# sidward14/gan-lab

Measured on AMD Instinct MI355X. Metric: images/sec (G+D step), StyleGAN 1024^2 bs32/GPU, higher is better.
Workload: dtype f32; 1 GPU; StyleGAN res_samples=1024 FFHQ-shaped synthetic, bs=32/GPU fp32, nonsaturating + R1(lambda=10) + drift, stabilised phase, 1 D-iter + 1 G-iter; global_batch=32, per_gpu_batch=32, parallelism=single

## Files before the change

### gan_lab_amd/csrc/common.h

```cpp
#pragma once
#include <hip/hip_runtime.h>
#include <stdint.h>

#include "../../include/ganlab_hip.h"

typedef float f32x4 __attribute__((ext_vector_type(4)));

static thread_local int gl_launch_status = GANLAB_OK;
extern thread_local const void* gl_last_kernel_fn;
extern thread_local unsigned gl_last_grid;
#define GL_LAUNCH_RING 16
extern thread_local const void* gl_ring_fn[GL_LAUNCH_RING];
extern thread_local unsigned gl_ring_grid[GL_LAUNCH_RING];
extern thread_local unsigned long long gl_launch_count;
#define GL_LAUNCH(k, grid, ...)                                                  \
  do {                                                                           \
    (void)hipGetLastError();                                                     \
    const dim3 gl_grid_ = (grid);                                                \
    gl_last_kernel_fn = reinterpret_cast<const void*>(k);                        \
    gl_last_grid = gl_grid_.x * gl_grid_.y * gl_grid_.z;                         \
    gl_ring_fn[gl_launch_count % GL_LAUNCH_RING] = gl_last_kernel_fn;            \
    gl_ring_grid[gl_launch_count % GL_LAUNCH_RING] = gl_last_grid;               \
    ++gl_launch_count;                                                           \
    hipLaunchKernelGGL(k, gl_grid_, __VA_ARGS__);                                \
    if (hipGetLastError() != hipSuccess) gl_launch_status = GANLAB_ELAUNCH;      \
  } while (0)
static inline int gl_take_status() {
  const int s = gl_launch_status;
  gl_launch_status = GANLAB_OK;
  return s;
}
#define GL_CHECK_LAUNCH() gl_take_status()

#include <cstdlib>
#define GL_ENV_ONCE(name) ([]() -> const char* { static const char* const v = getenv(name); return v; }())

static inline hipStream_t gl_stream(void* s) { return reinterpret_cast<hipStream_t>(s); }

__device__ __forceinline__ int gl_xcd_remap(int b, int n) {
  const int q = n >> 3, r = n & 7, xcd = b & 7, i = b >> 3;
  const int base = (xcd < r) ? xcd * (q + 1) : r * (q + 1) + (xcd - r) * q;
  return base + i;
}

__device__ __forceinline__ float gl_wave_sum(float v) {
#pragma unroll
  for (int o = 32; o > 0; o >>= 1) v += __shfl_xor(v, o, 64);
  return v;
}

__device__ __forceinline__ float gl_block_sum_256(float v, float* red) {
  v = gl_wave_sum(v);
  __syncthreads();
  if ((threadIdx.x & 63) == 0) red[threadIdx.x >> 6] = v;
  __syncthreads();
  return red[0] + red[1] + red[2] + red[3];
}

__device__ __forceinline__ double gl_block_sum_256d(double v, double* red) {
#pragma unroll
  for (int o = 32; o > 0; o >>= 1) v += __shfl_xor(v, o, 64);
  __syncthreads();
  if ((threadIdx.x & 63) == 0) red[threadIdx.x >> 6] = v;
  __syncthreads();
  return (red[0] + red[1]) + (red[2] + red[3]);
}

#ifndef GL_ACC_DUMP
#define GL_ACC_DUMP 1
#endif
#ifndef GL_ACC_DUMP_TERMS_V
#define GL_ACC_DUMP_TERMS_V 144
#endif
constexpr int GL_ACC_DUMP_TERMS = GL_ACC_DUMP_TERMS_V;

__device__ __forceinline__ void philox4x32_10(uint32_t c[4], uint32_t k0, uint32_t k1) {
#pragma unroll
  for (int r = 0; r < 10; ++r) {
    const uint64_t p0 = (uint64_t)0xD2511F53u * c[0], p1 = (uint64_t)0xCD9E8D57u * c[2];
    const uint32_t n0 = (uint32_t)(p1 >> 32) ^ c[1] ^ k0, n1 = (uint32_t)p1;
    const uint32_t n2 = (uint32_t)(p0 >> 32) ^ c[3] ^ k1, n3 = (uint32_t)p0;
    c[0] = n0; c[1] = n1; c[2] = n2; c[3] = n3;
    k0 += 0x9E3779B9u;
    k1 += 0xBB67AE85u;
  }
}

__device__ __forceinline__ float gl_lrelu(float v, float slope) { return v > 0.f ? v : v * slope; }

__device__ __forceinline__ float4 gl_few_dot(const float4 (&xv)[4], const float* __restrict__ wp, int Cin, int Cout_p, int co,
                                             float start) {
  float4 a = float4{start, start, start, start};
#pragma unroll
  for (int ci = 0; ci < 4; ++ci) {
    const float w = ci < Cin ? wp[(long long)ci * Cout_p + co] : 0.f;
    a.x += w * xv[ci].x; a.y += w * xv[ci].y; a.z += w * xv[ci].z; a.w += w * xv[ci].w;
  }
  return a;
}

struct gl_bf16x3 { __bf16 h, m, l; };
__device__ __forceinline__ gl_bf16x3 gl_split3(float v) {
  const __bf16 h = (__bf16)v;
  const float r1 = v - (float)h;
  const __bf16 m = (__bf16)r1;
  return gl_bf16x3{h, m, (__bf16)(r1 - (float)m)};
}

__device__ __forceinline__ void gl_x3_pack_position(const float* __restrict__ w9, bool flip, float scale, __bf16* __restrict__ out,
                                                    int CI, int ci, int co) {
  const int steps = CI / 32 * 9;
  const int ct = co >> 6, col = co & 63, c = ci >> 5, half = (ci >> 4) & 1, g = (ci >> 3) & 1, j = ci & 7;
#pragma unroll
  for (int t = 0; t < 9; ++t) {
    const int s = t < 8 ? (half ? 5 : 0) + (t >> 1) : 4;
    const int hi = t < 8 ? (t & 1) : half;
    const int kg = hi * 2 + g;
    float v = w9[flip ? 8 - t : t] * scale;
    asm volatile("" : "+v"(v));
    const gl_bf16x3 p = gl_split3(v);
    __bf16* base = out + (((long long)ct * steps + c * 9 + s) * (3 * 4 * 64)) * 8;
    base[((0 * 4 + kg) * 64 + col) * 8 + j] = p.h;
    base[((1 * 4 + kg) * 64 + col) * 8 + j] = p.m;
    base[((2 * 4 + kg) * 64 + col) * 8 + j] = p.l;
  }
}

__device__ __forceinline__ void gl_x3_up_pack_position(const float* __restrict__ w9, int up, float scale, __bf16* __restrict__ out,
                                                       int CI, int CO, int ci, int co) {
  const int nsteps = CI / 8;
  const bool c32 = (CO & 63) != 0;
  const int ct = c32 ? co >> 5 : co >> 6, j = ci & 7;
#pragma unroll
  for (int py = 0; py < 2; ++py)
#pragma unroll
    for (int px = 0; px < 2; ++px)
#pragma unroll
      for (int ty = 0; ty < 2; ++ty)
#pragma unroll
        for (int tx = 0; tx < 2; ++tx) {
          float v = 0.f;
#pragma unroll
          for (int ky = 0; ky < 3; ++ky)
#pragma unroll
            for (int kx = 0; kx < 3; ++kx) {
              const int ry = up ? ky : 2 - ky, rx = up ? kx : 2 - kx;
              const bool iny = py == 0 ? (ty == 0 ? ry == 0 : ry >= 1) : (ty == 0 ? ry <= 1 : ry == 2);
              const bool inx = px == 0 ? (tx == 0 ? rx == 0 : rx >= 1) : (tx == 0 ? rx <= 1 : rx == 2);
              if (iny && inx) v += w9[ky * 3 + kx];
            }
          v = v * (up ? scale : 0.25f * scale);
          asm volatile("" : "+v"(v));
          const gl_bf16x3 p = gl_split3(v);
          __bf16* base = out + (((c32 ? (long long)ct : (long long)ct * 2 + py) * nsteps + (ci >> 3)) * (3 * 4 * 128)) * 8;
          const int col = c32 ? py * 32 + (co & 31) : co & 63;
          const int kgq = ty * 2 + tx;
          base[((0 * 4 + kgq) * 128 + px * 64 + col) * 8 + j] = p.h;
          base[((1 * 4 + kgq) * 128 + px * 64 + col) * 8 + j] = p.m;
          base[((2 * 4 + kgq) * 128 + px * 64 + col) * 8 + j] = p.l;
        }
}

__device__ __forceinline__ float gl_comb_s2(int up, int a, int k) {
  if (up) {
    const int lo = (a == 0) ? 2 : (a == 1 ? 1 : 0), hi = (a == 0) ? 2 : (a == 1 ? 2 : (a == 2 ? 1 : 0));
    return (k >= lo && k <= hi) ? 1.f : 0.f;
  }
  const int lo = (a <= 1) ? 0 : (a == 2 ? 1 : 2), hi = (a == 0) ? 0 : (a == 1 ? 1 : 2);
  return (k >= lo && k <= hi) ? 0.5f : 0.f;
}
__device__ __forceinline__ void gl_x3_down_pack_position(const float* __restrict__ w9, int up, float scale, __bf16* __restrict__ out,
                                                         int CI, int ci, int co) {
  const int nsteps = CI / 8 * 4;
  const int ct = co >> 7, col = co & 127, q = ci >> 3, j = ci & 7;
  float k9[9];
#pragma unroll
  for (int t = 0; t < 9; ++t) k9[t] = w9[t];
#pragma unroll
  for (int a = 0; a < 4; ++a)
#pragma unroll
    for (int b = 0; b < 4; ++b) {
      float v = 0.f;
#pragma unroll
      for (int ky = 0; ky < 3; ++ky)
#pragma unroll
        for (int kx = 0; kx < 3; ++kx) v += gl_comb_s2(up, a, ky) * gl_comb_s2(up, b, kx) * k9[ky * 3 + kx];
      v = v * scale;
      asm volatile("" : "+v"(v));
      const gl_bf16x3 p = gl_split3(v);
      __bf16* base = out + (((long long)ct * nsteps + q * 4 + a) * (3 * 4 * 128)) * 8;
      base[((0 * 4 + b) * 128 + col) * 8 + j] = p.h;
      base[((1 * 4 + b) * 128 + col) * 8 + j] = p.m;
      base[((2 * 4 + b) * 128 + col) * 8 + j] = p.l;
    }
}

extern "C" int gl_tail_stats_finish(const double* spart, float* mean, float* rstd, long long planes, int chunks, double inv_hw, float eps,
                         hipStream_t st);

bool gl_wgrad_roll_supported(int N, int Cin, int Cout, int H, int W, int ks, int pad, int up, const void* x,
                             const void* gy);
int gl_wgrad_roll_slots(int N, int Cin, int Cout, int H, int W);
int gl_wgrad_roll_launch(const float* x, const float* gy, float* part, int N, int Cin, int Cout, int H, int W,
                         hipStream_t st, const float* aff_s = nullptr, const float* aff_t = nullptr);
bool gl_wgrad_s2_roll_supported(int N, int Cl, int Ch, int Hl, int Wl, const void* low, const void* high);
int gl_wgrad_s2_roll_slots(int N, int Cl, int Ch, int Hl, int Wl);
int gl_wgrad_s2_roll_launch(const float* low, const float* high, float* part, int N, int Cl, int Ch, int Hl, int Wl,
                            hipStream_t st, const float* aff_s = nullptr, const float* aff_t = nullptr);

bool gl_s2_roll_supported(int is_T, int N, int Cin, int Cout, int Hl, int Wl, const void* x, const void* y);
int gl_s2_roll_launch(int is_T, const float* x, const float* wp, const float* bias, float* y, int N, int Cin, int Cout,
                      int Hl, int Wl, int Cin_p, int Cout_p, float bias_scale, int act, float slope, hipStream_t st,
                      const float* aff_s = nullptr, const float* aff_t = nullptr);

bool gl_roll_blur_supported(int N, int Cin, int Cout, int H, int W, const void* x, const void* y);
int gl_roll_blur_launch(const float* x, const float* wp, const float* bias, float* y, void* bits, int N, int Cin, int Cout,
                        int H, int W, int Cin_p, int Cout_p, float bias_scale, float slope, hipStream_t st, int blur, int act);
```

### gan_lab_amd/csrc/conv_x3_down.hip

```cpp
#include "x3_common.h"

#include <type_traits>

namespace {

constexpr int XD_NT = 128;
constexpr int XD_PP = 160;
constexpr int XD_PL = 4 * XD_PP;
constexpr int XD_Q = 3 * XD_PL;
constexpr int XD_WSTEP = 3 * 4 * XD_NT;
constexpr int XD_WOFF = 3 * XD_Q;
constexpr int XD_LDS = 3 * XD_Q + 2 * XD_WSTEP;

#define XD_ACC8(a) "+v"(a[0][0]), "+v"(a[0][1]), "+v"(a[0][2]), "+v"(a[0][3]), "+v"(a[1][0]), "+v"(a[1][1]), "+v"(a[1][2]), "+v"(a[1][3])

struct XDArgs {
  const float* x;
  const u32x4* wp;
  const float* bias;
  float* y;
  int N, CI, CO, Hl, Wl;
  int tiles_x, tiles_y, tiles_co, ntiles;
  float bias_scale, slope;
  int act;
};
struct XDTile { int n, oy0, ox0, co_t; };

__global__ __launch_bounds__(512) void conv_x3_down_kernel(XDArgs p) {
  __shared__ __attribute__((aligned(16))) u32x4 lds[XD_LDS];
  const int tid = threadIdx.x, lane = tid & 63;
  const int wv = __builtin_amdgcn_readfirstlane(tid >> 6);
  const int wm = wv >> 1, wn = wv & 1;
  const int l16 = lane & 15, kg = lane >> 4, lane16 = lane * 16;
  const int Hi = 2 * p.Hl, Wi = 2 * p.Wl;
  const int plane = Hi * Wi;
  const int oplane = p.Hl * p.Wl;
  const int nq = p.CI / 8;
  const int G = gridDim.x;

  auto decode = [&](int t) {
    XDTile c;
    c.co_t = t % p.tiles_co; t /= p.tiles_co;
    c.ox0 = (t % p.tiles_x) * 16; t /= p.tiles_x;
    c.oy0 = (t % p.tiles_y) * 8;
    c.n = t / p.tiles_y;
    return c;
  };

  const bool a_item = tid < 360;
  int a_r, a_cg, a_cq;
  {
    const int e = a_item ? tid : 0;
    a_cq = e & 1;
    const int t = e >> 1;
    a_cg = t % 10;
    a_r = t / 10;
  }
  const int cstride = plane * 4;
  f32x4 arA[4], arB[4];
  auto a_load_to = [&](f32x4 (&ar)[4], const XDTile& c, int q) {
    const u32x4 rs = x3_rsrc(p.x + (long long)c.n * p.CI * plane, (unsigned)((long long)p.CI * plane * 4));
    int r = a_r;
    asm volatile("" : "+v"(r));
    const int iy = 2 * c.oy0 - 1 + r, ix = 2 * c.ox0 - 4 + 4 * a_cg;
    const bool ok = a_item && (unsigned)iy < (unsigned)Hi && (unsigned)ix < (unsigned)Wi;
    const int off = ok ? ((a_cq * 4) * plane + iy * Wi + ix) * 4 : (int)0x80000000;
    const int soff = q * 8 * plane * 4;
#pragma unroll
    for (int j = 0; j < 4; ++j) x3_ld(ar[j], rs, off + j * cstride, soff);
  };
  auto a_store_from = [&](const f32x4 (&ar)[4], int slot, int i) {
    if (!a_item) return;
    int r = a_r;
    asm volatile("" : "+v"(r));
    const int c = 4 * a_cg - 3 + i;
    if (c < 0 || c > 33) return;
    bf16x4 h, m, l;
#pragma unroll
    for (int j = 0; j < 4; ++j) x3_split_lane(ar[j][i], j, h, m, l);
    const int unit = slot * XD_Q + ((r & 1) * 2 + (c & 1)) * XD_PP + (r >> 1) * 17 + (c >> 1);
    unsigned char* dst = reinterpret_cast<unsigned char*>(lds + unit) + a_cq * 8;
    *reinterpret_cast<u32x2*>(dst) = __builtin_bit_cast(u32x2, h);
    *reinterpret_cast<u32x2*>(dst + XD_PL * 16) = __builtin_bit_cast(u32x2, m);
    *reinterpret_cast<u32x2*>(dst + 2 * XD_PL * 16) = __builtin_bit_cast(u32x2, l);
  };
  auto a_load = [&](int set, const XDTile& c, int q) { if (set == 0) a_load_to(arA, c, q); else a_load_to(arB, c, q); };
  auto a_store_px = [&](int set, int slot, int i) { if (set == 0) a_store_from(arA, slot, i); else a_store_from(arB, slot, i); };
  auto a_wait = [&](int set, auto younger) {
    constexpr int Y = decltype(younger)::value;
    if (set == 0) x3_ld_wait<Y>(arA); else x3_ld_wait<Y>(arB);
  };

  const int nsteps = nq * 4;
  const __amdgpu_buffer_rsrc_t rs_w = __builtin_amdgcn_make_buffer_rsrc(
      const_cast<u32x4*>(p.wp), 0, (unsigned)((long long)p.tiles_co * nsteps * XD_WSTEP * 16), 0x00020000);
  auto w_dma = [&](const XDTile& c, int step, int buf) {
    const int soff = (c.co_t * nsteps + step) * (XD_WSTEP * 16) + wv * 3072;
#pragma unroll
    for (int i = 0; i < 3; ++i)
      __builtin_amdgcn_raw_ptr_buffer_load_lds(rs_w, (__attribute__((address_space(3))) void*)(lds + XD_WOFF + buf * XD_WSTEP + wv * 192 + i * 64),
                                               16, lane16, soff + i * 1024, 0, 0);
  };

  f32x4 accS[2][4], accH[2][4], accT[2][4];
#pragma unroll
  for (int m = 0; m < 2; ++m)
#pragma unroll
    for (int nn = 0; nn < 4; ++nn) {
      accS[m][nn] = f32x4{0.f, 0.f, 0.f, 0.f}; accH[m][nn] = f32x4{0.f, 0.f, 0.f, 0.f}; accT[m][nn] = f32x4{0.f, 0.f, 0.f, 0.f};
    }
  X3_SETTLE(XD_ACC8(accS));
  X3_SETTLE(XD_ACC8(accH));

  const int laneA = (kg & 1) * XD_PP + (2 * wm) * 17 + l16 + (kg >> 1);
  const int laneB = XD_WOFF + kg * XD_NT + wn * 64 + l16;

  bf16x8 aF[2][2][3];
  bf16x8 bF[2][3];
  auto a_frags = [&](int off, int set) {
#pragma unroll
    for (int m = 0; m < 2; ++m)
#pragma unroll
      for (int pl = 0; pl < 3; ++pl) aF[set][m][pl] = __builtin_bit_cast(bf16x8, lds[laneA + off + pl * XD_PL + m * 17]);
  };
  auto b_frags = [&](int buf, int nn, int set) {
#pragma unroll
    for (int pl = 0; pl < 3; ++pl) bF[set][pl] = __builtin_bit_cast(bf16x8, lds[laneB + buf * XD_WSTEP + pl * 4 * XD_NT + nn * 16]);
  };

  int tile = gl_xcd_remap(blockIdx.x, G);
  if (tile >= p.ntiles) return;
  XDTile cur = decode(tile);
  int sa = 0, sb = 1, sc = 2;

  w_dma(cur, 0, 0);
  a_load(0, cur, 0);
  a_wait(0, std::integral_constant<int, 0>{});
#pragma unroll
  for (int i = 0; i < 4; ++i) { a_store_px(0, sa, i); __builtin_amdgcn_sched_barrier(0); }
  x3_barrier<0>();
  w_dma(cur, 1, 1);
  __builtin_amdgcn_sched_barrier(0);
  a_load(1, cur, 1);
  a_wait(1, std::integral_constant<int, 0>{});
  a_frags(sa * XD_Q, 0);
  b_frags(0, 0, 0);

  int q = 0, gs = 0;
  for (;;) {
    const int ntile = tile + G;
    const bool nvalid = ntile < p.ntiles;
    const XDTile nxt = decode(nvalid ? ntile : tile);
    for (; q < nq; q += 2) {
#pragma unroll
      for (int s8 = 0; s8 < 8; ++s8) {
        const int qq = q + (s8 >> 2), a = s8 & 3;
        const int buf = (gs + s8) & 1, cs = s8 & 1;
        const int setn = (s8 >> 2) ^ 1;
        const bool has_next = a < 3 || qq + 1 < nq || nvalid;
        const bool next_q = qq + 1 < nq || nvalid;
        const int offN = a < 3 ? sa * XD_Q + ((a + 1) & 1) * 2 * XD_PP + ((a + 1) >> 1) * 17 : sb * XD_Q;
#pragma unroll
        for (int nn = 0; nn < 4; ++nn) {
          if (nn < 3) b_frags(buf, nn + 1, (nn + 1) & 1);
          if (nn == 3) {
            if (a == 1 && (qq + 2 < nq || nvalid)) x3_barrier<4>(); else x3_barrier<0>();
            {
              const int st2 = qq * 4 + a + 2;
              if (st2 < nsteps) w_dma(cur, st2, buf);
              else if (nvalid) w_dma(nxt, st2 - nsteps, buf);
            }
            __builtin_amdgcn_sched_barrier(0);
            if (a == 0) {
              if (qq + 2 < nq) a_load(setn ^ 1, cur, qq + 2);
              else if (nvalid) a_load(setn ^ 1, nxt, qq + 2 - nq);
            }
            if (has_next) { a_frags(offN, cs ^ 1); b_frags(buf ^ 1, 0, 0); }
          }
          __builtin_amdgcn_sched_barrier(0);
#pragma unroll
          for (int m = 0; m < 2; ++m) {
            X3_MFMA(accS[m][nn], aF[cs][m][2], bF[nn & 1][0]);
            X3_MFMA(accS[m][nn], aF[cs][m][0], bF[nn & 1][2]);
            X3_MFMA(accS[m][nn], aF[cs][m][1], bF[nn & 1][1]);
            X3_MFMA(accS[m][nn], aF[cs][m][1], bF[nn & 1][0]);
            X3_MFMA(accS[m][nn], aF[cs][m][0], bF[nn & 1][1]);
            X3_MFMA(accH[m][nn], aF[cs][m][0], bF[nn & 1][0]);
          }
          __builtin_amdgcn_sched_barrier(0);
          if (nn == 1 && next_q) {
            if (a == 0) a_wait(setn, std::integral_constant<int, 9>{});
            a_store_px(setn, sb, a);
            __builtin_amdgcn_sched_barrier(0);
          }
        }
        if (a == 3) { const int t_ = sa; sa = sb; sb = sc; sc = t_; }
      }
      gs += 8;
      X3_DRAIN(XD_ACC8(accH));
#pragma unroll
      for (int m = 0; m < 2; ++m)
#pragma unroll
        for (int nn = 0; nn < 4; ++nn) { accT[m][nn] += accH[m][nn]; accH[m][nn] = f32x4{0.f, 0.f, 0.f, 0.f}; }
      X3_SETTLE(XD_ACC8(accH));
      __builtin_amdgcn_sched_barrier(0);
    }

    {
      X3_DRAIN(XD_ACC8(accS));
      typedef const __attribute__((address_space(4))) XDArgs* XDArgsK;
      unsigned long long kpi = (unsigned long long)__builtin_amdgcn_kernarg_segment_ptr();
      asm volatile("" : "+s"(kpi));
      const XDArgsK kp = (XDArgsK)kpi;
      float* const y = kp->y;
      const float* const bias = kp->bias;
      const float bias_scale = kp->bias_scale, slope = kp->slope;
      const int act = kp->act;
      const long long ib = (long long)cur.n * p.CO * oplane;
#pragma unroll
      for (int nn = 0; nn < 4; ++nn) {
        const int co = cur.co_t * XD_NT + wn * 64 + nn * 16 + l16;
        const float bv = bias != nullptr ? bias[co] * bias_scale : 0.f;
#pragma unroll
        for (int m = 0; m < 2; ++m) {
          f32x4 v = accT[m][nn] + accS[m][nn];
#pragma unroll
          for (int r = 0; r < 4; ++r) {
            float f = v[r] + bv;
            if (act == GANLAB_ACT_LRELU) f = gl_lrelu(f, slope);
            v[r] = f;
          }
          *reinterpret_cast<f32x4*>(y + ib + (long long)co * oplane + (cur.oy0 + 2 * wm + m) * p.Wl + cur.ox0 + 4 * kg) = v;
          accT[m][nn] = f32x4{0.f, 0.f, 0.f, 0.f};
          accS[m][nn] = f32x4{0.f, 0.f, 0.f, 0.f};
        }
      }
      X3_SETTLE(XD_ACC8(accS));
    }
    if (!nvalid) break;
    tile = ntile;
    cur = nxt;
    q = 0;
  }
}

__global__ void x3_down_pack_kernel(const float* __restrict__ w, __bf16* __restrict__ out, int Cout, int Cin, int up, float scale) {
  const int CO = up ? Cin : Cout, CI = up ? Cout : Cin;
  const long long e = blockIdx.x * (long long)blockDim.x + threadIdx.x;
  if (e >= (long long)CO * CI) return;
  const int col = (int)(e & 127);
  const long long t = e >> 7;
  const int ci = (int)(t % CI), ct = (int)(t / CI);
  const int co = ct * 128 + col;
  const float* w9 = up ? w + ((long long)ci * Cin + co) * 9 : w + ((long long)co * Cin + ci) * 9;
  gl_x3_down_pack_position(w9, up, scale, out, CI, ci, co);
}

long long xd_tiles(int N, int CI, int CO, int Hl, int Wl) {
  const long long ntiles = (long long)N * (Wl / 16) * (Hl / 8) * (CO / XD_NT);
  const bool fits = ntiles > 0 && ntiles <= 0x7fffffffLL && (long long)(CO / XD_NT) * (CI / 8 * 4) * XD_WSTEP * 16 <= 0xffffffffLL &&
                    (long long)CI * Hl * Wl * 16 <= 0x7fffffffLL;
  return fits ? ntiles : 0;
}

bool xd_ok(const ganlab_conv_geom* g, int dgrad) {
  if (g == nullptr || g->ks != 3 || g->pad != 1 || g->N <= 0) return false;
  if (dgrad ? !(g->up == 1 && g->pool == 0) : !(g->pool == 1 && g->up == 0)) return false;
  const int CI = dgrad ? g->Cout : g->Cin, CO = dgrad ? g->Cin : g->Cout;
  if (!dgrad && ((g->Hin | g->Win) & 1)) return false;
  const int Hl = dgrad ? g->Hin : g->Hin / 2, Wl = dgrad ? g->Win : g->Win / 2;
  if (!(CI % 16 == 0 && CO % XD_NT == 0 && Hl % 8 == 0 && Wl % 16 == 0)) return false;
  return xd_tiles(g->N, CI, CO, Hl, Wl) > 0;
}

int xd_launch(const float* x, const void* wp, const float* bias, float* y, int N, int CI, int CO, int Hl, int Wl, float bias_scale,
              int act, float slope, hipStream_t st) {
  XDArgs a{};
  a.x = x; a.wp = reinterpret_cast<const u32x4*>(wp); a.bias = bias; a.y = y;
  a.N = N; a.CI = CI; a.CO = CO; a.Hl = Hl; a.Wl = Wl;
  a.tiles_x = Wl / 16; a.tiles_y = Hl / 8; a.tiles_co = CO / XD_NT;
  a.bias_scale = bias_scale; a.slope = slope; a.act = act;
  const long long ntiles = xd_tiles(N, CI, CO, Hl, Wl);
  if (ntiles <= 0) return GANLAB_EINVAL;
  a.ntiles = (int)ntiles;
  const unsigned grid = (unsigned)(ntiles < 256 ? ntiles : 256);
  GL_LAUNCH(conv_x3_down_kernel, dim3(grid), dim3(512), 0, st, a);
  return GL_CHECK_LAUNCH();
}

}

extern "C" {

int ganlab_conv_s2_down_x3_supported(const ganlab_conv_geom* g, int dgrad) { return xd_ok(g, dgrad) ? 1 : 0; }

long long ganlab_conv_s2_down_x3_pack(const float* w, void* out, int Cout, int Cin, int up, float scale, void* stream) {
  if (Cout <= 0 || Cin <= 0 || (up != 0 && up != 1)) return GANLAB_EINVAL;
  const int CO = up ? Cin : Cout, CI = up ? Cout : Cin;
  if (CO % XD_NT != 0 || CI % 16 != 0) return GANLAB_EINVAL;
  const long long n = 48LL * Cout * Cin;
  if (out == nullptr) return n;
  if (w == nullptr) return GANLAB_EINVAL;
  const long long positions = (long long)Cout * Cin;
  GL_LAUNCH(x3_down_pack_kernel, dim3((unsigned)((positions + 255) / 256)), dim3(256), 0, gl_stream(stream), w,
            reinterpret_cast<__bf16*>(out), Cout, Cin, up, scale);
  const int st = GL_CHECK_LAUNCH();
  return st != GANLAB_OK ? st : n;
}

int ganlab_conv_s2_down_fwd_x3(const float* x, const void* wp, const float* bias, float* y, const ganlab_conv_geom* g,
                               float bias_scale, int act, float slope, void* stream) {
  if (!xd_ok(g, 0) || x == nullptr || wp == nullptr || y == nullptr) return GANLAB_EINVAL;
  return xd_launch(x, wp, bias, y, g->N, g->Cin, g->Cout, g->Hin / 2, g->Win / 2, bias_scale, act, slope, gl_stream(stream));
}

int ganlab_conv_s2_down_dgrad_x3(const float* gy, const void* wp, float* gx, const ganlab_conv_geom* g, void* stream) {
  if (!xd_ok(g, 1) || gy == nullptr || wp == nullptr || gx == nullptr) return GANLAB_EINVAL;
  return xd_launch(gy, wp, nullptr, gx, g->N, g->Cout, g->Cin, g->Hin, g->Win, 1.f, GANLAB_ACT_NONE, 0.f, gl_stream(stream));
}

}
```

### gan_lab_amd/csrc/pack.hip

```cpp
#include "common.h"

namespace {

constexpr int round_up_c(int v, int m) { return (v + m - 1) / m * m; }

__global__ __launch_bounds__(256) void pack_many_kernel(const ganlab_pack_desc* __restrict__ descs, int n_desc) {
  int lo = 0, hi = n_desc - 1;
  const long long b = blockIdx.x;
  while (lo < hi) {
    const int mid = (lo + hi + 1) >> 1;
    if (descs[mid].block0 <= b) lo = mid; else hi = mid - 1;
  }
  const ganlab_pack_desc d = descs[lo];
  const long long e = (b - d.block0) * 256 + threadIdx.x;
  const float* w = d.src;
  if (d.kind == GANLAB_PACKKIND_PLAIN) {
    const int KK = d.ks * d.ks, dgrad = d.mode == GANLAB_PACK_DGRAD;
    const int rows = dgrad ? d.Cout : d.Cin, cols = dgrad ? d.Cin : d.Cout;
    const int rows_p = round_up_c(rows, d.ks == 1 ? 32 : 16), cols_p = round_up_c(cols, 64);
    const long long plane = (long long)rows_p * cols_p;
    if (e >= plane) return;
    const int col = (int)(e % cols_p), row = (int)(e / cols_p);
    const bool in = row < rows && col < cols;
    const int co = dgrad ? row : col, ci = dgrad ? col : row;
    const float* ws = w + ((long long)co * d.Cin + ci) * KK;
    float* out = reinterpret_cast<float*>(d.dst) + e;
    for (int tap = 0; tap < KK; ++tap)
      out[tap * plane] = in ? d.scale * ws[dgrad ? (KK - 1 - tap) : tap] : 0.f;
  } else if (d.kind == GANLAB_PACKKIND_S2) {
    const int transpose = d.mode;
    const int rows = transpose ? d.Cout : d.Cin, cols = transpose ? d.Cin : d.Cout;
    const int rows_p = round_up_c(rows, 16), cols_p = round_up_c(cols, 64);
    const long long plane = (long long)rows_p * cols_p;
    if (e >= plane) return;
    const int col = (int)(e % cols_p), row = (int)(e / cols_p);
    const bool in = row < rows && col < cols;
    const int co = transpose ? row : col, ci = transpose ? col : row;
    float k9[9];
    const float* ws = w + ((long long)co * d.Cin + ci) * 9;
#pragma unroll
    for (int t = 0; t < 9; ++t) k9[t] = in ? ws[t] : 0.f;
    float* out = reinterpret_cast<float*>(d.dst) + e;
#pragma unroll
    for (int tap = 0; tap < 16; ++tap) {
      const int a = tap >> 2, bb = tap & 3;
      float v = 0.f;
#pragma unroll
      for (int ky = 0; ky < 3; ++ky)
#pragma unroll
        for (int kx = 0; kx < 3; ++kx) v += gl_comb_s2(d.up, a, ky) * gl_comb_s2(d.up, bb, kx) * k9[ky * 3 + kx];
      out[tap * plane] = v * d.scale;
    }
  } else if (d.kind == GANLAB_PACKKIND_X3 && d.ks == 4) {
    const int up = d.up;
    const int CO = up ? d.Cout : d.Cin, CI = up ? d.Cin : d.Cout;
    if (e >= (long long)CO * CI) return;
    int ci, co;
    if ((CO & 63) == 0) {
      const int col = (int)(e & 63);
      const long long t = e >> 6;
      ci = (int)(t % CI);
      co = (int)(t / CI) * 64 + col;
    } else {
      co = (int)(e % CO);
      ci = (int)(e / CO);
    }
    const float* w9 = up ? w + ((long long)co * d.Cin + ci) * 9 : w + ((long long)ci * d.Cin + co) * 9;
    gl_x3_up_pack_position(w9, up, d.scale, reinterpret_cast<__bf16*>(d.dst), CI, CO, ci, co);
  } else if (d.kind == GANLAB_PACKKIND_X3 && d.ks == 5) {
    const int up = d.up;
    const int CO = up ? d.Cin : d.Cout, CI = up ? d.Cout : d.Cin;
    if (e >= (long long)CO * CI) return;
    const int col = (int)(e & 127);
    const long long t = e >> 7;
    const int ci = (int)(t % CI), ct = (int)(t / CI);
    const int co = ct * 128 + col;
    const float* w9 = up ? w + ((long long)ci * d.Cin + co) * 9 : w + ((long long)co * d.Cin + ci) * 9;
    gl_x3_down_pack_position(w9, up, d.scale, reinterpret_cast<__bf16*>(d.dst), CI, ci, co);
  } else if (d.kind == GANLAB_PACKKIND_X3) {
    const bool dg = d.mode == GANLAB_PACK_DGRAD;
    const int CO = dg ? d.Cin : d.Cout, CI = dg ? d.Cout : d.Cin;
    if (e >= (long long)CO * CI) return;
    const int col = (int)(e & 63);
    const long long t = e >> 6;
    const int ci = (int)(t % CI), ct = (int)(t / CI);
    const int co = ct * 64 + col;
    const float* w9 = dg ? w + ((long long)ci * d.Cin + co) * 9 : w + ((long long)co * d.Cin + ci) * 9;
    gl_x3_pack_position(w9, dg, d.scale, reinterpret_cast<__bf16*>(d.dst), CI, ci, co);
  } else {
    const int dg = d.mode == GANLAB_PACK_DGRAD;
    const int CO = dg ? d.Cin : d.Cout;
    if (e >= d.total / 9) return;
    const int j = (int)(e & 7);
    long long t = e >> 3;
    const int co = (int)(t % CO);
    t /= CO;
    const int kg = (int)(t & 3);
    const int chunk = (int)(t >> 2);
    const int ci = chunk * 32 + kg * 8 + j;
    const float* ws = dg ? w + ((long long)ci * d.Cin + co) * 9 : w + ((long long)co * d.Cin + ci) * 9;
    __bf16* out = reinterpret_cast<__bf16*>(d.dst);
#pragma unroll
    for (int tap = 0; tap < 9; ++tap)
      out[((((long long)chunk * 9 + tap) * 4 + kg) * CO + co) * 8 + j] = (__bf16)(ws[dg ? 8 - tap : tap] * d.scale);
  }
}

}

extern "C" {

int ganlab_pack_desc_size(void) { return (int)sizeof(ganlab_pack_desc); }

int ganlab_pack_many(const ganlab_pack_desc* descs_device, int n_desc, long long total_blocks, void* stream) {
  if (!descs_device || n_desc <= 0 || total_blocks <= 0 || total_blocks > 0x7fffffffLL) return GANLAB_EINVAL;
  GL_LAUNCH(pack_many_kernel, dim3((unsigned)total_blocks), dim3(256), 0, gl_stream(stream), descs_device, n_desc);
  return GL_CHECK_LAUNCH();
}

}
```

### gan_lab_amd/ops.py

```python
import ctypes
import os

import numpy as np

import torch
from torch.autograd import Function
from torch.autograd.function import once_differentiable

from . import _lib
from ._lib import ACT_LRELU, ACT_NONE, PACK_DGRAD, PACK_FWD, ConvGeom, check


def _p(t):
    return ctypes.c_void_p(t.data_ptr()) if t is not None else None


_RAW_STREAM = getattr(torch._C, '_cuda_getCurrentRawStream', None)
_GET_DEVICE = getattr(torch._C, '_cuda_getDevice', None)


def _st():
    if _RAW_STREAM is None or _GET_DEVICE is None:
        return ctypes.c_void_p(torch.cuda.current_stream().cuda_stream)
    return ctypes.c_void_p(_RAW_STREAM(_GET_DEVICE()))
# ... 209 lines not shown
        return
    if tab is None or tab[0] != keys:
        arr = (_lib.PackDesc * len(items))()
        blocks = 0
        for i, (_, e) in enumerate(items):
            kind, cout, cin, ks, mode, up, scale, total = e.desc
            d = arr[i]
            d.src, d.dst = e.w.data_ptr(), e.out.data_ptr()
            d.kind, d.Cout, d.Cin, d.ks, d.mode, d.up, d.scale, d.total, d.block0 = kind, cout, cin, ks, mode, up, scale, \
                total, blocks
            blocks += (total // (16 if kind == _KIND_S2 else (9 if kind == _KIND_BF16 else ((48 if ks >= 4 else 27) if kind == _KIND_X3 else ks * ks))) + 255) // 256
        host = torch.frombuffer(bytearray(bytes(arr)), dtype=torch.uint8)
        if tab is not None:
            _PACK_GEN[0] += 1
        tab = (keys, host.to(items[0][1].w.device), blocks)
        _PACK_TABLES[r] = tab
    check(L.ganlab_pack_many(tab[1].data_ptr(), len(items), tab[2], _st()), 'pack_many')
    now = _PACK_SERIAL[0]
    for _, e in items:
        e.serial = now


def _pack_lookup(key):
    e = _PACK_CACHE.get(key)
    if e is None:
        return None
    r = _stale_range(e)
    if r is not None:
        _repack_range(r)
    return e.out


def _pack_store(key, w, out, desc):
    if len(_PACK_CACHE) > 1024:
        bump_weight_epoch()
    e = _PackEntry()
    e.w, e.out, e.serial, e.ptr, e.desc = w.detach(), out, _PACK_SERIAL[0], w.data_ptr(), desc
    _PACK_CACHE[key] = e
    return out


def _packed(w, mode, scale, s2_up=None):
    key = (w.data_ptr(), w._version, tuple(w.shape), mode, float(scale), s2_up)
    hit = _pack_lookup(key)
    if hit is not None:
        return hit
    cout, cin, ks = w.shape[0], w.shape[1], w.shape[2]
    L = _lib.lib()
    if s2_up is not None:
        tr = 1 if mode == PACK_DGRAD else 0
        n = L.ganlab_conv_s2_pack_f32(None, None, cout, cin, int(s2_up), tr, scale, None)
        if n <= 0:
            raise _lib.GanlabLibraryError(f'conv_s2_pack size query failed ({n}) for weight {tuple(w.shape)}')
        out = _new((n,), w)
        rc = L.ganlab_conv_s2_pack_f32(_p(w), _p(out), cout, cin, int(s2_up), tr, scale, _st())
        if rc != n:
            raise _lib.GanlabLibraryError(f'conv_s2_pack failed ({rc})')
        return _pack_store(key, w, out, (_KIND_S2, cout, cin, 3, tr, int(s2_up), float(scale), int(n)))
    n = L.ganlab_conv_pack_f32(None, None, cout, cin, ks, mode, scale, None)
    if n <= 0:
        raise _lib.GanlabLibraryError(f'conv_pack size query failed ({n}) for weight {tuple(w.shape)}')
    out = _new((n,), w)
    rc = L.ganlab_conv_pack_f32(_p(w), _p(out), cout, cin, ks, mode, scale, _st())
    if rc != n:
        raise _lib.GanlabLibraryError(f'conv_pack failed ({rc})')
    return _pack_store(key, w, out, (_KIND_PLAIN, cout, cin, ks, mode, 0, float(scale), int(n)))


def _packed_bf16(w, mode, scale):
    key = (w.data_ptr(), w._version, tuple(w.shape), mode, float(scale), 'bf16')
    hit = _pack_lookup(key)
    if hit is not None:
        return hit
    cout, cin = w.shape[0], w.shape[1]
    L = _lib.lib()
    n = L.ganlab_conv_pack_bf16(None, None, cout, cin, mode, scale, None)
    if n <= 0:
        raise _lib.GanlabLibraryError(f'conv_pack_bf16 size query failed ({n}) for weight {tuple(w.shape)}')
    out = torch.empty((n,), dtype=torch.bfloat16, device=w.device)
    rc = L.ganlab_conv_pack_bf16(_p(w), out.data_ptr(), cout, cin, mode, scale, _st())
    if rc != n:
        raise _lib.GanlabLibraryError(f'conv_pack_bf16 failed ({rc})')
    return _pack_store(key, w, out, (_KIND_BF16, cout, cin, 3, mode, 0, float(scale), int(n)))


_X3 = [os.environ.get('GANLAB_X3', '1') != '0']
_X3_MIN_TILES = 128


def set_x3(enabled):
    old = _X3[0]
    _X3[0] = bool(enabled)
    return old


def x3_enabled():
    return _X3[0]


def x3_ok(g, dgrad=False):
    if not _X3[0] or g.bf is not None or g.s2 or g.up or g.pool or g.ks != 3 or g.pad != 1:
        return False
    co = g.Cin if dgrad else g.Cout
    if g.N * (g.Hin // 16) * (g.Win // 16) * (co // 64) < _X3_MIN_TILES:
        return False
    return bool(_lib.lib().ganlab_conv_x3_supported(g.ref(), 1 if dgrad else 0))


def x3_s2_ok(g, dgrad=False):
    if not _X3[0] or not g.s2:
        return False
    if (g.pool if dgrad else g.up) != 1:
        return False
    co = g.Cin if dgrad else g.Cout
    hl, wl = (g.Hin // 2, g.Win // 2) if dgrad else (g.Hin, g.Win)
    if g.N * (hl // 8) * (wl // 16) * (co // 32) < _X3_MIN_TILES:
        return False
    return bool(_lib.lib().ganlab_conv_s2_x3_supported(g.ref(), 1 if dgrad else 0))


def x3_wgrad_ok(g):
    if not _X3[0] or g.bf is not None or g.s2 or g.up or g.pool or g.ks != 3 or g.pad != 1 or g.Cin < 64 or g.Cout < 64:
        return False
    return bool(_lib.lib().ganlab_conv_wgrad_x3_supported(g.ref()))


def _wgrad_x3(gy, x, s_, t_, gw, g, scale):
    L = _lib.lib()
    ws = torch.empty((L.ganlab_conv_wgrad_x3_workspace(g.ref()) + 3) // 4, dtype=torch.float32, device=x.device)
    check(L.ganlab_conv_wgrad_x3(_p(gy), _p(x), _p(s_), _p(t_), _p(gw), g.ref(), scale, _p(ws), ws.numel() * 4, _st()),
          'conv_wgrad_x3')
    return gw


def x3_s2_wgrad_ok(g):
    if not _X3[0] or g.bf is not None or not g.s2 or g.ks != 3 or g.pad != 1:
        return False
    return bool(_lib.lib().ganlab_conv_s2_wgrad_x3_supported(g.ref()))


def _wgrad_x3_s2(gy, x, s_, t_, gw, g, scale):
    L = _lib.lib()
    ws = torch.empty((L.ganlab_conv_s2_wgrad_x3_workspace(g.ref()) + 3) // 4, dtype=torch.float32, device=x.device)
    check(L.ganlab_conv_s2_wgrad_x3(_p(gy), _p(x), _p(s_), _p(t_), _p(gw), g.ref(), scale, _p(ws), ws.numel() * 4, _st()),
          'conv_s2_wgrad_x3')
    return gw


def x3_s2_down_ok(g, dgrad=False):
    if not _X3[0] or not g.s2:
        return False
    if (g.up if dgrad else g.pool) != 1:
        return False
    co = g.Cin if dgrad else g.Cout
    hl, wl = (g.Hin, g.Win) if dgrad else (g.Hin // 2, g.Win // 2)
    if g.N * (hl // 8) * (wl // 16) * (co // 128) < _X3_MIN_TILES:
        return False
    return bool(_lib.lib().ganlab_conv_s2_down_x3_supported(g.ref(), 1 if dgrad else 0))


def _packed_x3_any(name, tag, w, sel, scale, ks):
    key = (w.data_ptr(), w._version, tuple(w.shape), sel, float(scale), tag)
    hit = _pack_lookup(key)
    if hit is not None:
        return hit
    cout, cin = w.shape[0], w.shape[1]
    pack = getattr(_lib.lib(), 'ganlab_' + name)
    n = pack(None, None, cout, cin, sel, scale, None)
    if n <= 0:
        raise _lib.GanlabLibraryError(f'{name} size query failed ({n}) for weight {tuple(w.shape)}')
    out = torch.empty((n,), dtype=torch.bfloat16, device=w.device)
    rc = pack(_p(w), out.data_ptr(), cout, cin, sel, scale, _st())
    if rc != n:
        raise _lib.GanlabLibraryError(f'{name} failed ({rc})')
    mode, up = (sel, 0) if ks == 3 else (0, sel)
    return _pack_store(key, w, out, (_KIND_X3, cout, cin, ks, mode, up, float(scale), int(n)))


def _packed_x3_s2_down(w, up, scale):
    return _packed_x3_any('conv_s2_down_x3_pack', 'x3s2d', w, int(up), scale, 5)


def _packed_x3_s2(w, up, scale):
    return _packed_x3_any('conv_s2_x3_pack', 'x3s2', w, int(up), scale, 4)


def _packed_x3(w, mode, scale):
    return _packed_x3_any('conv_x3_pack', 'x3', w, mode, scale, 3)


_INPUT_GRAD_ONLY = [False]


class input_grad_only(object):
    def __enter__(self):
        self._prev = _INPUT_GRAD_ONLY[0]
        _INPUT_GRAD_ONLY[0] = True

    def __exit__(self, *exc):
        _INPUT_GRAD_ONLY[0] = self._prev
        return False


def _want_param_grads():
    return not _INPUT_GRAD_ONLY[0]


_NO_GRAD_TOWARDS = [None]


class no_grad_towards(object):
    def __init__(self, leaf):
        self.ptr = leaf.data_ptr() if leaf is not None else None

    def __enter__(self):
        self._prev = _NO_GRAD_TOWARDS[0]
        _NO_GRAD_TOWARDS[0] = self.ptr

    def __exit__(self, *exc):
        _NO_GRAD_TOWARDS[0] = self._prev
        return False


def _wants_input_grad(ctx, x):
    return ctx.needs_input_grad[0] and not (_NO_GRAD_TOWARDS[0] is not None and x.grad_fn is None and
                                            x.data_ptr() == _NO_GRAD_TOWARDS[0])


_DIRECT = [False]
_SINK, _TAKEN = {}, {}


def direct_grads_enabled():
    import os
    return os.environ.get('GANLAB_DIRECT_GRADS') != '0'


class direct_param_grads(object):
    def __init__(self, enabled=True):
        self.enabled = bool(enabled)

    def __enter__(self):
        self._prev = _DIRECT[0]
        _DIRECT[0] = self.enabled
        _SINK.clear()
        _TAKEN.clear()

    def __exit__(self, *exc):
        _DIRECT[0] = self._prev
        _SINK.clear()
        _TAKEN.clear()
        return False


def _sink(name, p):
    if not _DIRECT[0] or p is None or torch.is_grad_enabled():
        return
    base = p._base if p._base is not None else p
    arena = getattr(base, '_ganlab_arena', None)
    if arena is None or not base.is_leaf or base.grad is None or base.numel() != p.numel() or \
            getattr(base, '_ganlab_written', -1) == arena.serial:
        return
    _SINK[name] = base


def _take(name, shape, like):
    if _SINK:
        base = _SINK.pop(name, None)
        if base is not None:
            n = 1
            for v in shape:
                n *= int(v)
            if base.grad.numel() == n and base.grad.device == like.device:
                base._ganlab_written = base._ganlab_arena.serial
                _TAKEN[name] = True
                return base.grad.view(shape)
    return _new(shape, like)


def _sunk(name):
    if _SINK:
        _SINK.pop(name, None)
    return _TAKEN.pop(name, False) if _TAKEN else False


_OBSERVER = [None]


def set_launch_observer(fn):
    prev = _OBSERVER[0]
    _OBSERVER[0] = fn
    return prev


def conv_flops(g):
    if g.s2:
        lo_h, lo_w = (g.Hin, g.Win) if g.up else (g.Ho, g.Wo)
        return 2.0 * 16 * g.Cin * g.Cout * lo_h * lo_w * g.N
    if g.bf is not None:
        return 2.0 * g.ks * g.ks * g.Cin * g.Cout * g.bf.Hin * g.bf.Win * g.N
    return 2.0 * g.ks * g.ks * g.Cin * g.Cout * g.Ho * g.Wo * g.N


def _note(kind, g):
    if _OBSERVER[0] is not None:
        _OBSERVER[0](kind, g)


def k_conv_fwd(x, w, bias, g, scale, bias_scale=1.0, act=ACT_NONE, slope=0.2):
    x, w = _c(x, 'conv input'), _c(w, 'conv weight')
    assert tuple(x.shape) == g.in_shape, (tuple(x.shape), g.in_shape)
# ... 4209 lines not shown
```

Before: 168.7 images/sec.

## Extend strided-down x3 conv kernel to 64 and 32 output-channel widths

Templates the bf16x3 split MFMA strided-down convolution on output-channel tile width (128, 64, 32). Narrow widths get their own weight pack layout, DMA pattern and K-step schedule, and a cross-wave LDS reduction in the epilogue. This lets the high-resolution layers with 32/64 channels (StyleGAN D at 1024/512) use the MFMA path instead of a fallback. One 16-to-32 large-plane case stays excluded. It adds template complexity and new layout risk.

New measurement: 169.3 images/sec (median of 6 runs). About the same (+0.4%).

```diff
diff --git a/gan_lab_amd/csrc/common.h b/gan_lab_amd/csrc/common.h
--- a/gan_lab_amd/csrc/common.h
+++ b/gan_lab_amd/csrc/common.h
@@ -169,8 +169,20 @@
   const int lo = (a <= 1) ? 0 : (a == 2 ? 1 : 2), hi = (a == 0) ? 0 : (a == 1 ? 1 : 2);
   return (k >= lo && k <= hi) ? 0.5f : 0.f;
 }
+__device__ __forceinline__ void gl_x3_down_pack_index(long long e, int CO, int CI, int& ci, int& co) {
+  if ((CO & 127) == 0) {
+    const int col = (int)(e & 127);
+    const long long t = e >> 7;
+    ci = (int)(t % CI);
+    co = (int)(t / CI) * 128 + col;
+  } else {
+    co = (int)(e % CO);
+    ci = (int)(e / CO);
+  }
+}
 __device__ __forceinline__ void gl_x3_down_pack_position(const float* __restrict__ w9, int up, float scale, __bf16* __restrict__ out,
-                                                         int CI, int ci, int co) {
+                                                         int CI, int CO, int ci, int co) {
+  const bool narrow = (CO & 127) != 0;
   const int nsteps = CI / 8 * 4;
   const int ct = co >> 7, col = co & 127, q = ci >> 3, j = ci & 7;
   float k9[9];
@@ -188,10 +200,12 @@
       v = v * scale;
       asm volatile("" : "+v"(v));
       const gl_bf16x3 p = gl_split3(v);
-      __bf16* base = out + (((long long)ct * nsteps + q * 4 + a) * (3 * 4 * 128)) * 8;
-      base[((0 * 4 + b) * 128 + col) * 8 + j] = p.h;
-      base[((1 * 4 + b) * 128 + col) * 8 + j] = p.m;
-      base[((2 * 4 + b) * 128 + col) * 8 + j] = p.l;
+      const int W = narrow ? CO : 128;
+      __bf16* base = narrow ? out + ((long long)((q * 2 + (a >> 1)) * 2 + (a & 1)) * (3 * 4 * W)) * 8
+                            : out + (((long long)ct * nsteps + q * 4 + a) * (3 * 4 * 128)) * 8;
+      base[((0 * 4 + b) * W + col) * 8 + j] = p.h;
+      base[((1 * 4 + b) * W + col) * 8 + j] = p.m;
+      base[((2 * 4 + b) * W + col) * 8 + j] = p.l;
     }
 }
 
diff --git a/gan_lab_amd/csrc/conv_x3_down.hip b/gan_lab_amd/csrc/conv_x3_down.hip
--- a/gan_lab_amd/csrc/conv_x3_down.hip
+++ b/gan_lab_amd/csrc/conv_x3_down.hip
@@ -11,6 +11,8 @@
 constexpr int XD_WSTEP = 3 * 4 * XD_NT;
 constexpr int XD_WOFF = 3 * XD_Q;
 constexpr int XD_LDS = 3 * XD_Q + 2 * XD_WSTEP;
+constexpr int xd_wstep(int CW) { return CW == 128 ? XD_WSTEP : 2 * 3 * 4 * CW; }
+constexpr int xd_lds(int CW) { return 3 * XD_Q + 2 * xd_wstep(CW) + (CW == 64 ? 128 : 0); }
 
 #define XD_ACC8(a) "+v"(a[0][0]), "+v"(a[0][1]), "+v"(a[0][2]), "+v"(a[0][3]), "+v"(a[1][0]), "+v"(a[1][1]), "+v"(a[1][2]), "+v"(a[1][3])
 
@@ -26,8 +28,15 @@
 };
 struct XDTile { int n, oy0, ox0, co_t; };
 
+template <int CW>
 __global__ __launch_bounds__(512) void conv_x3_down_kernel(XDArgs p) {
-  __shared__ __attribute__((aligned(16))) u32x4 lds[XD_LDS];
+  static_assert(CW == 128 || CW == 64 || CW == 32, "output channels of a workgroup");
+  constexpr bool NARROW = CW != 128;
+  constexpr int NB = NARROW ? CW / 16 : 4;
+  constexpr int KS = NARROW ? 2 : 4;
+  constexpr int WSTEP = xd_wstep(CW);
+  constexpr int NDMA = WSTEP / 512;
+  __shared__ __attribute__((aligned(16))) u32x4 lds[xd_lds(CW)];
   const int tid = threadIdx.x, lane = tid & 63;
   const int wv = __builtin_amdgcn_readfirstlane(tid >> 6);
   const int wm = wv >> 1, wn = wv & 1;
@@ -91,15 +100,24 @@
     if (set == 0) x3_ld_wait<Y>(arA); else x3_ld_wait<Y>(arB);
   };
 
-  const int nsteps = nq * 4;
+  const int nsteps = nq * KS;
   const __amdgpu_buffer_rsrc_t rs_w = __builtin_amdgcn_make_buffer_rsrc(
-      const_cast<u32x4*>(p.wp), 0, (unsigned)((long long)p.tiles_co * nsteps * XD_WSTEP * 16), 0x00020000);
+      const_cast<u32x4*>(p.wp), 0, (unsigned)((long long)p.tiles_co * nsteps * WSTEP * 16), 0x00020000);
   auto w_dma = [&](const XDTile& c, int step, int buf) {
-    const int soff = (c.co_t * nsteps + step) * (XD_WSTEP * 16) + wv * 3072;
-#pragma unroll
-    for (int i = 0; i < 3; ++i)
-      __builtin_amdgcn_raw_ptr_buffer_load_lds(rs_w, (__attribute__((address_space(3))) void*)(lds + XD_WOFF + buf * XD_WSTEP + wv * 192 + i * 64),
-                                               16, lane16, soff + i * 1024, 0, 0);
+    if constexpr (CW != 32) {
+      const int soff = (c.co_t * nsteps + step) * (WSTEP * 16) + wv * 3072;
+#pragma unroll
+      for (int i = 0; i < 3; ++i)
+        __builtin_amdgcn_raw_ptr_buffer_load_lds(rs_w, (__attribute__((address_space(3))) void*)(lds + XD_WOFF + buf * WSTEP + wv * 192 + i * 64),
+                                                 16, lane16, soff + i * 1024, 0, 0);
+    } else {
+      const int soff = (c.co_t * nsteps + step) * (WSTEP * 16) + wv * 1024;
+      __builtin_amdgcn_raw_ptr_buffer_load_lds(rs_w, (__attribute__((address_space(3))) void*)(lds + XD_WOFF + buf * WSTEP + wv * 64),
+                                               16, lane16, soff, 0, 0);
+      if (wv < 4)
+        __builtin_amdgcn_raw_ptr_buffer_load_lds(rs_w, (__attribute__((address_space(3))) void*)(lds + XD_WOFF + buf * WSTEP + (wv + 8) * 64),
+                                                 16, lane16, soff + 8192, 0, 0);
+    }
   };
 
   f32x4 accS[2][4], accH[2][4], accT[2][4];
@@ -113,7 +131,8 @@
   X3_SETTLE(XD_ACC8(accH));
 
   const int laneA = (kg & 1) * XD_PP + (2 * wm) * 17 + l16 + (kg >> 1);
-  const int laneB = XD_WOFF + kg * XD_NT + wn * 64 + l16;
+  const int laneB = NARROW ? XD_WOFF + wn * (3 * 4 * CW) + kg * CW + l16 : XD_WOFF + kg * XD_NT + wn * 64 + l16;
+  const int rowA = NARROW ? wn * 2 * XD_PP : 0;
 
   bf16x8 aF[2][2][3];
   bf16x8 bF[2][3];
@@ -125,7 +144,7 @@
   };
   auto b_frags = [&](int buf, int nn, int set) {
 #pragma unroll
-    for (int pl = 0; pl < 3; ++pl) bF[set][pl] = __builtin_bit_cast(bf16x8, lds[laneB + buf * XD_WSTEP + pl * 4 * XD_NT + nn * 16]);
+    for (int pl = 0; pl < 3; ++pl) bF[set][pl] = __builtin_bit_cast(bf16x8, lds[laneB + buf * WSTEP + pl * 4 * CW + nn * 16]);
   };
 
   int tile = gl_xcd_remap(blockIdx.x, G);
@@ -143,7 +162,7 @@
   __builtin_amdgcn_sched_barrier(0);
   a_load(1, cur, 1);
   a_wait(1, std::integral_constant<int, 0>{});
-  a_frags(sa * XD_Q, 0);
+  a_frags(sa * XD_Q + rowA, 0);
   b_frags(0, 0, 0);
 
   int q = 0, gs = 0;
@@ -153,20 +172,21 @@
     const XDTile nxt = decode(nvalid ? ntile : tile);
     for (; q < nq; q += 2) {
 #pragma unroll
-      for (int s8 = 0; s8 < 8; ++s8) {
-        const int qq = q + (s8 >> 2), a = s8 & 3;
+      for (int s8 = 0; s8 < 2 * KS; ++s8) {
+        const int qq = q + s8 / KS, a = s8 % KS;
         const int buf = (gs + s8) & 1, cs = s8 & 1;
-        const int setn = (s8 >> 2) ^ 1;
-        const bool has_next = a < 3 || qq + 1 < nq || nvalid;
+        const int setn = (s8 / KS) ^ 1;
+        const bool has_next = a < KS - 1 || qq + 1 < nq || nvalid;
         const bool next_q = qq + 1 < nq || nvalid;
-        const int offN = a < 3 ? sa * XD_Q + ((a + 1) & 1) * 2 * XD_PP + ((a + 1) >> 1) * 17 : sb * XD_Q;
-#pragma unroll
-        for (int nn = 0; nn < 4; ++nn) {
-          if (nn < 3) b_frags(buf, nn + 1, (nn + 1) & 1);
-          if (nn == 3) {
+        const int offN = NARROW ? (a < KS - 1 ? sa * XD_Q + rowA + (a + 1) * 17 : sb * XD_Q + rowA)
+                                : (a < 3 ? sa * XD_Q + ((a + 1) & 1) * 2 * XD_PP + ((a + 1) >> 1) * 17 : sb * XD_Q);
+#pragma unroll
+        for (int nn = 0; nn < NB; ++nn) {
+          if (nn < NB - 1) b_frags(buf, nn + 1, (nn + 1) & 1);
+          if (nn == NB - 1) {
             if (a == 1 && (qq + 2 < nq || nvalid)) x3_barrier<4>(); else x3_barrier<0>();
             {
-              const int st2 = qq * 4 + a + 2;
+              const int st2 = qq * KS + a + 2;
               if (st2 < nsteps) w_dma(cur, st2, buf);
               else if (nvalid) w_dma(nxt, st2 - nsteps, buf);
             }
@@ -188,15 +208,27 @@
             X3_MFMA(accH[m][nn], aF[cs][m][0], bF[nn & 1][0]);
           }
           __builtin_amdgcn_sched_barrier(0);
-          if (nn == 1 && next_q) {
-            if (a == 0) a_wait(setn, std::integral_constant<int, 9>{});
-            a_store_px(setn, sb, a);
-            __builtin_amdgcn_sched_barrier(0);
+          if constexpr (!NARROW) {
+            if (nn == 1 && next_q) {
+              if (a == 0) a_wait(setn, std::integral_constant<int, 9>{});
+              a_store_px(setn, sb, a);
+              __builtin_amdgcn_sched_barrier(0);
+            }
+          } else {
+            if (nn == NB / 2 - 1 && next_q) {
+              if (a == 0 && (s8 > 0 || q > 0)) a_wait(setn, std::integral_constant<int, NDMA>{});
+              a_store_px(setn, sb, 2 * a);
+              __builtin_amdgcn_sched_barrier(0);
+            }
+            if (nn == (NB == 2 ? 0 : NB / 2) && next_q) {
+              a_store_px(setn, sb, 2 * a + 1);
+              __builtin_amdgcn_sched_barrier(0);
+            }
           }
         }
-        if (a == 3) { const int t_ = sa; sa = sb; sb = sc; sc = t_; }
+        if (a == KS - 1) { const int t_ = sa; sa = sb; sb = sc; sc = t_; }
       }
-      gs += 8;
+      gs += 2 * KS;
       X3_DRAIN(XD_ACC8(accH));
 #pragma unroll
       for (int m = 0; m < 2; ++m)
@@ -217,23 +249,57 @@
       const float bias_scale = kp->bias_scale, slope = kp->slope;
       const int act = kp->act;
       const long long ib = (long long)cur.n * p.CO * oplane;
-#pragma unroll
-      for (int nn = 0; nn < 4; ++nn) {
-        const int co = cur.co_t * XD_NT + wn * 64 + nn * 16 + l16;
-        const float bv = bias != nullptr ? bias[co] * bias_scale : 0.f;
-#pragma unroll
-        for (int m = 0; m < 2; ++m) {
-          f32x4 v = accT[m][nn] + accS[m][nn];
+      if constexpr (NARROW) {
+        if (nvalid) a_wait(1, std::integral_constant<int, NDMA>{});
+        auto xunit = [&](int nn, int w_) -> u32x4* {
+          const int e = (nn * 8 + w_) * 64 + lane;
+          return (CW == 64 && nn == 3 && w_ >= 6) ? lds + (3 * XD_Q + 2 * WSTEP - XD_Q) + e : lds + sc * XD_Q + e;
+        };
+#pragma unroll
+        for (int nn = 0; nn < NB; ++nn) {
+          const f32x4 give = wn == 0 ? accT[1][nn] + accS[1][nn] : accT[0][nn] + accS[0][nn];
+          *xunit(nn, wv) = __builtin_bit_cast(u32x4, give);
+        }
+        asm volatile("s_waitcnt lgkmcnt(0)\n\ts_barrier" ::: "memory");
+#pragma unroll
+        for (int nn = 0; nn < NB; ++nn) {
+          const int co = nn * 16 + l16;
+          const float bv = bias != nullptr ? bias[co] * bias_scale : 0.f;
+          const f32x4 mine = wn == 0 ? accT[0][nn] + accS[0][nn] : accT[1][nn] + accS[1][nn];
+          const f32x4 got = __builtin_bit_cast(f32x4, *xunit(nn, wv ^ 1));
+          f32x4 v = wn == 0 ? mine + got : got + mine;
 #pragma unroll
           for (int r = 0; r < 4; ++r) {
             float f = v[r] + bv;
             if (act == GANLAB_ACT_LRELU) f = gl_lrelu(f, slope);
             v[r] = f;
           }
+          *reinterpret_cast<f32x4*>(y + ib + (long long)co * oplane + (cur.oy0 + 2 * wm + wn) * p.Wl + cur.ox0 + 4 * kg) = v;
+#pragma unroll
+          for (int m = 0; m < 2; ++m) {
+            accT[m][nn] = f32x4{0.f, 0.f, 0.f, 0.f};
+            accS[m][nn] = f32x4{0.f, 0.f, 0.f, 0.f};
+          }
+        }
+      } else {
+#pragma unroll
+      for (int nn = 0; nn < 4; ++nn) {
+        const int co = cur.co_t * XD_NT + wn * 64 + nn * 16 + l16;
+        const float bv = bias != nullptr ? bias[co] * bias_scale : 0.f;
+#pragma unroll
+        for (int m = 0; m < 2; ++m) {
+          f32x4 v = accT[m][nn] + accS[m][nn];
+#pragma unroll
+          for (int r = 0; r < 4; ++r) {
+            float f = v[r] + bv;
+            if (act == GANLAB_ACT_LRELU) f = gl_lrelu(f, slope);
+            v[r] = f;
+          }
           *reinterpret_cast<f32x4*>(y + ib + (long long)co * oplane + (cur.oy0 + 2 * wm + m) * p.Wl + cur.ox0 + 4 * kg) = v;
           accT[m][nn] = f32x4{0.f, 0.f, 0.f, 0.f};
           accS[m][nn] = f32x4{0.f, 0.f, 0.f, 0.f};
         }
+      }
       }
       X3_SETTLE(XD_ACC8(accS));
     }
@@ -248,17 +314,19 @@
   const int CO = up ? Cin : Cout, CI = up ? Cout : Cin;
   const long long e = blockIdx.x * (long long)blockDim.x + threadIdx.x;
   if (e >= (long long)CO * CI) return;
-  const int col = (int)(e & 127);
-  const long long t = e >> 7;
-  const int ci = (int)(t % CI), ct = (int)(t / CI);
-  const int co = ct * 128 + col;
+  int ci, co;
+  gl_x3_down_pack_index(e, CO, CI, ci, co);
   const float* w9 = up ? w + ((long long)ci * Cin + co) * 9 : w + ((long long)co * Cin + ci) * 9;
-  gl_x3_down_pack_position(w9, up, scale, out, CI, ci, co);
-}
+  gl_x3_down_pack_position(w9, up, scale, out, CI, CO, ci, co);
+}
+
+int xd_width(int CO) { return CO > 0 && CO % XD_NT == 0 ? XD_NT : (CO == 64 || CO == 32) ? CO : 0; }
 
 long long xd_tiles(int N, int CI, int CO, int Hl, int Wl) {
-  const long long ntiles = (long long)N * (Wl / 16) * (Hl / 8) * (CO / XD_NT);
-  const bool fits = ntiles > 0 && ntiles <= 0x7fffffffLL && (long long)(CO / XD_NT) * (CI / 8 * 4) * XD_WSTEP * 16 <= 0xffffffffLL &&
+  const int cw = xd_width(CO);
+  if (cw == 0) return 0;
+  const long long ntiles = (long long)N * (Wl / 16) * (Hl / 8) * (CO / cw);
+  const bool fits = ntiles > 0 && ntiles <= 0x7fffffffLL && (long long)(CO / cw) * (CI / 8 * 4) * (3 * 4 * cw) * 16 <= 0xffffffffLL &&
                     (long long)CI * Hl * Wl * 16 <= 0x7fffffffLL;
   return fits ? ntiles : 0;
 }
@@ -269,7 +337,7 @@
   const int CI = dgrad ? g->Cout : g->Cin, CO = dgrad ? g->Cin : g->Cout;
   if (!dgrad && ((g->Hin | g->Win) & 1)) return false;
   const int Hl = dgrad ? g->Hin : g->Hin / 2, Wl = dgrad ? g->Win : g->Win / 2;
-  if (!(CI % 16 == 0 && CO % XD_NT == 0 && Hl % 8 == 0 && Wl % 16 == 0)) return false;
+  if (!(CI > 0 && CI % 16 == 0 && xd_width(CO) != 0 && Hl % 8 == 0 && Wl % 16 == 0)) return false;
   return xd_tiles(g->N, CI, CO, Hl, Wl) > 0;
 }
 
@@ -278,13 +346,17 @@
   XDArgs a{};
   a.x = x; a.wp = reinterpret_cast<const u32x4*>(wp); a.bias = bias; a.y = y;
   a.N = N; a.CI = CI; a.CO = CO; a.Hl = Hl; a.Wl = Wl;
-  a.tiles_x = Wl / 16; a.tiles_y = Hl / 8; a.tiles_co = CO / XD_NT;
+  const int cw = xd_width(CO);
+  if (cw == 0 || CI <= 0 || CI % 16 != 0) return GANLAB_EINVAL;
+  a.tiles_x = Wl / 16; a.tiles_y = Hl / 8; a.tiles_co = CO / cw;
   a.bias_scale = bias_scale; a.slope = slope; a.act = act;
   const long long ntiles = xd_tiles(N, CI, CO, Hl, Wl);
   if (ntiles <= 0) return GANLAB_EINVAL;
   a.ntiles = (int)ntiles;
   const unsigned grid = (unsigned)(ntiles < 256 ? ntiles : 256);
-  GL_LAUNCH(conv_x3_down_kernel, dim3(grid), dim3(512), 0, st, a);
+  if (cw == 128) GL_LAUNCH(conv_x3_down_kernel<128>, dim3(grid), dim3(512), 0, st, a);
+  else if (cw == 64) GL_LAUNCH(conv_x3_down_kernel<64>, dim3(grid), dim3(512), 0, st, a);
+  else GL_LAUNCH(conv_x3_down_kernel<32>, dim3(grid), dim3(512), 0, st, a);
   return GL_CHECK_LAUNCH();
 }
 
@@ -297,7 +369,7 @@
 long long ganlab_conv_s2_down_x3_pack(const float* w, void* out, int Cout, int Cin, int up, float scale, void* stream) {
   if (Cout <= 0 || Cin <= 0 || (up != 0 && up != 1)) return GANLAB_EINVAL;
   const int CO = up ? Cin : Cout, CI = up ? Cout : Cin;
-  if (CO % XD_NT != 0 || CI % 16 != 0) return GANLAB_EINVAL;
+  if (xd_width(CO) == 0 || CI % 16 != 0) return GANLAB_EINVAL;
   const long long n = 48LL * Cout * Cin;
   if (out == nullptr) return n;
   if (w == nullptr) return GANLAB_EINVAL;
diff --git a/gan_lab_amd/csrc/pack.hip b/gan_lab_amd/csrc/pack.hip
--- a/gan_lab_amd/csrc/pack.hip
+++ b/gan_lab_amd/csrc/pack.hip
@@ -71,12 +71,10 @@
     const int up = d.up;
     const int CO = up ? d.Cin : d.Cout, CI = up ? d.Cout : d.Cin;
     if (e >= (long long)CO * CI) return;
-    const int col = (int)(e & 127);
-    const long long t = e >> 7;
-    const int ci = (int)(t % CI), ct = (int)(t / CI);
-    const int co = ct * 128 + col;
+    int ci, co;
+    gl_x3_down_pack_index(e, CO, CI, ci, co);
     const float* w9 = up ? w + ((long long)ci * d.Cin + co) * 9 : w + ((long long)co * d.Cin + ci) * 9;
-    gl_x3_down_pack_position(w9, up, d.scale, reinterpret_cast<__bf16*>(d.dst), CI, ci, co);
+    gl_x3_down_pack_position(w9, up, d.scale, reinterpret_cast<__bf16*>(d.dst), CI, CO, ci, co);
   } else if (d.kind == GANLAB_PACKKIND_X3) {
     const bool dg = d.mode == GANLAB_PACK_DGRAD;
     const int CO = dg ? d.Cin : d.Cout, CI = dg ? d.Cout : d.Cin;
diff --git a/gan_lab_amd/ops.py b/gan_lab_amd/ops.py
--- a/gan_lab_amd/ops.py
+++ b/gan_lab_amd/ops.py
@@ -385,11 +385,17 @@
         return False
     if (g.up if dgrad else g.pool) != 1:
         return False
-    co = g.Cin if dgrad else g.Cout
+    ci, co = (g.Cout, g.Cin) if dgrad else (g.Cin, g.Cout)
     hl, wl = (g.Hin, g.Win) if dgrad else (g.Hin // 2, g.Win // 2)
-    if g.N * (hl // 8) * (wl // 16) * (co // 128) < _X3_MIN_TILES:
+    cw = 128 if co % 128 == 0 else co
+    if g.N * (hl // 8) * (wl // 16) * (co // cw) < _X3_MIN_TILES:
+        return False
+    if ci == 16 and co == 32 and hl * wl >= _X3_DOWN_ROLL_MIN_PLANE:
         return False
     return bool(_lib.lib().ganlab_conv_s2_down_x3_supported(g.ref(), 1 if dgrad else 0))
+
+
+_X3_DOWN_ROLL_MIN_PLANE = 256 * 256
 
 
 def _packed_x3_any(name, tag, w, sel, scale, ks):
```
